# BarryFutureman/EvolutionaryDistributedTraining

Hardware: AMD Instinct MI355X
Metric: GB/s of param bytes reduced per outer step (device-resident), 1/2/4/8 GPUs (higher is better)
Workload: dtype f32; 1 GPU; DiLoCo outer step, gpt_1p3b P=1315723264 T=292, population 8 (8 f32 workers resident per GPU), f32 theta+momentum, lr 0.7 mu 0.9 nesterov True; params=1315723264, tensors=292, workers_per_gpu=8, population=8, worker_dtype=f32, theta_dtype=f32, parallelism=single GPU

## Files before the change

evolutionarydistributedtraining_amd/csrc/edt_common.h:

```cpp
#pragma once

#include <hip/hip_runtime.h>
#include <stdarg.h>
#include <stdint.h>
#include <stdio.h>
#include <string.h>

#include <type_traits>
#include <vector>

#include "edt_sync.h"

namespace edt {
extern thread_local char g_err[512];
}

namespace {
using edt::g_err;


#ifndef EDT_BLOCKS_PER_CU
#define EDT_BLOCKS_PER_CU 0
#endif
#ifndef EDT_NT_LOADS
#define EDT_NT_LOADS 1
#endif
#ifndef EDT_NT_RMW
#define EDT_NT_RMW 0
#endif
#ifndef EDT_NT_STORES
#define EDT_NT_STORES 0
#endif

#ifndef EDT_NT_LERP
#define EDT_NT_LERP 0
#endif
#ifndef EDT_NT_LERP_STORES
#define EDT_NT_LERP_STORES 1
#endif
#ifndef EDT_NT_SLERP_STORES
#define EDT_NT_SLERP_STORES 1
#endif
#ifndef EDT_NT_SLERP
#define EDT_NT_SLERP 1
#endif
#ifndef EDT_SLERP_STATS_TPW
#define EDT_SLERP_STATS_TPW 16
#endif
#ifndef EDT_GRAM_NT
#define EDT_GRAM_NT 1
#endif
#ifndef EDT_NEED_GROUP
#define EDT_NEED_GROUP 8
#endif
#ifndef EDT_NEED_MIN_WAVES
#define EDT_NEED_MIN_WAVES 1
#endif
#ifndef EDT_NEED_GLDS
#define EDT_NEED_GLDS 1
#endif
#ifndef EDT_SLERP_SPEC_WG_ROWS
#define EDT_SLERP_SPEC_WG_ROWS 1
#endif
#ifndef EDT_SLERP_COEF_BLOCK
#define EDT_SLERP_COEF_BLOCK 1
#endif
#ifndef EDT_SPLIT_HALVES
#define EDT_SPLIT_HALVES 2
#endif
#ifndef EDT_NT_F32
#define EDT_NT_F32 1
#endif
template <int WDT, int H2>
constexpr bool nt_worker_loads() {
    return EDT_NT_LOADS != 0 && (WDT == EDT_BF16 || (EDT_NT_F32 != 0 && H2 != 4));
}

template <int GDT, int WDT>
constexpr bool split_halves() {
    return EDT_SPLIT_HALVES == 1 || (EDT_SPLIT_HALVES == 2 && GDT == EDT_F32 && WDT == EDT_F32);
}
#ifndef EDT_MIN_WAVES
#define EDT_MIN_WAVES 1
#endif

constexpr int kBlock = 256;
constexpr int kVec = 8;
constexpr uint64_t kGridBlockCap = 0xffffffffull / kBlock;
constexpr uint64_t kMaxBlocks = EDT_BLOCKS_PER_CU > 0 ? 256ull * EDT_BLOCKS_PER_CU : kGridBlockCap;

#ifndef EDT_XCD_RUN
#define EDT_XCD_RUN 0
#endif
__device__ __forceinline__ uint64_t xcd_block(uint64_t b, uint64_t G) {
    if constexpr (EDT_XCD_RUN == 0) {
        return b;
    } else {
        const uint64_t M = EDT_XCD_RUN > 0 ? (uint64_t)EDT_XCD_RUN : G / 8;
        const uint64_t span = 8 * M;
        if (M == 0 || b >= G / span * span) return b;
        const uint64_t g = b / span, x = b % 8, j = (b / 8) % M;
        return g * span + x * M + j;
    }
}

#ifndef EDT_SLERP_SPEC_BPC
#define EDT_SLERP_SPEC_BPC 256
#endif
inline unsigned slerp_spec_grid(int64_t nchunks) {
    const uint64_t cap = 256ull * EDT_SLERP_SPEC_BPC;
    return (unsigned)((uint64_t)nchunks < cap ? (uint64_t)nchunks : cap);
}
typedef float f32x4 __attribute__((ext_vector_type(4)));
typedef float f32x2 __attribute__((ext_vector_type(2)));
typedef uint32_t u32x4 __attribute__((ext_vector_type(4)));
typedef uint32_t u32x2 __attribute__((ext_vector_type(2)));
typedef __bf16 bf16x2 __attribute__((ext_vector_type(2)));



inline int fail(int code, const char* fmt, ...) {
    va_list ap;
    va_start(ap, fmt);
    vsnprintf(g_err, sizeof(g_err), fmt, ap);
    va_end(ap);
    return code;
}

inline int check_launch(const char* what) {
    hipError_t e = hipGetLastError();
    if (e != hipSuccess) return fail(EDT_ERR_LAUNCH, "%s: launch failed: %s", what, hipGetErrorString(e));
    return EDT_OK;
}


__device__ __forceinline__ float bf_lo(uint32_t w) { return __uint_as_float(w << 16); }
__device__ __forceinline__ float bf_hi(uint32_t w) { return __uint_as_float(w & 0xffff0000u); }
__device__ __forceinline__ uint32_t pack_bf(float lo, float hi) {
    bf16x2 r = __builtin_convertvector((f32x2){lo, hi}, bf16x2);
    return __builtin_bit_cast(uint32_t, r);
}
__host__ __device__ inline float host_round_bf16(float x) {
    uint32_t u;
    memcpy(&u, &x, 4);
    if ((u & 0x7fffffffu) > 0x7f800000u) return x;
    u = (u + 0x7fffu + ((u >> 16) & 1u)) & 0xffff0000u;
    float r;
    memcpy(&r, &u, 4);
    return r;
}

template <int DT, int N>
__device__ __forceinline__ void rnd(float (&x)[N]) {
    if constexpr (DT == EDT_BF16) {
        if constexpr (N % 2 == 0) {
#pragma unroll
            for (int j = 0; j < N; j += 2) {
                uint32_t p = pack_bf(x[j], x[j + 1]);
                x[j] = bf_lo(p);
                x[j + 1] = bf_hi(p);
            }
        } else {
#pragma unroll
            for (int j = 0; j < N; ++j) x[j] = bf_lo(pack_bf(x[j], 0.f));
        }
    }
}

template <typename V, bool NT>
__device__ __forceinline__ V vload(const V* p) {
    if constexpr (NT) return __builtin_nontemporal_load(p);
    else return *p;
}
template <typename V, bool NT>
__device__ __forceinline__ void vstore(V* p, V v) {
    if constexpr (NT) __builtin_nontemporal_store(v, p);
    else *p = v;
}

template <int DT, int N, bool NT = false, int H2 = 4>
__device__ __forceinline__ void ld(const void* __restrict__ p, uint64_t i, float (&x)[N]) {
    if constexpr (DT == EDT_F32) {
        const float* q = static_cast<const float*>(p) + i;
        if constexpr (N == 8) {
            f32x4 a = vload<f32x4, NT>(reinterpret_cast<const f32x4*>(q));
            f32x4 b = vload<f32x4, NT>(reinterpret_cast<const f32x4*>(q + H2));
            x[0] = a.x; x[1] = a.y; x[2] = a.z; x[3] = a.w;
            x[4] = b.x; x[5] = b.y; x[6] = b.z; x[7] = b.w;
        } else {
#pragma unroll
            for (int j = 0; j < N; ++j) x[j] = q[j];
        }
    } else {
        const uint16_t* q = static_cast<const uint16_t*>(p) + i;
        if constexpr (N == 8 && H2 == 4) {
            u32x4 w = vload<u32x4, NT>(reinterpret_cast<const u32x4*>(q));
            x[0] = bf_lo(w.x); x[1] = bf_hi(w.x); x[2] = bf_lo(w.y); x[3] = bf_hi(w.y);
            x[4] = bf_lo(w.z); x[5] = bf_hi(w.z); x[6] = bf_lo(w.w); x[7] = bf_hi(w.w);
        } else if constexpr (N == 8) {
            u32x2 w0 = vload<u32x2, NT>(reinterpret_cast<const u32x2*>(q));
            u32x2 w1 = vload<u32x2, NT>(reinterpret_cast<const u32x2*>(q + H2));
            x[0] = bf_lo(w0.x); x[1] = bf_hi(w0.x); x[2] = bf_lo(w0.y); x[3] = bf_hi(w0.y);
            x[4] = bf_lo(w1.x); x[5] = bf_hi(w1.x); x[6] = bf_lo(w1.y); x[7] = bf_hi(w1.y);
        } else {
#pragma unroll
            for (int j = 0; j < N; ++j) x[j] = __uint_as_float(uint32_t(q[j]) << 16);
        }
    }
}

template <int DT, int N, bool NT = (EDT_NT_STORES != 0), int H2 = 4>
__device__ __forceinline__ void st(void* __restrict__ p, uint64_t i, const float (&x)[N]) {
    if constexpr (DT == EDT_F32) {
        float* q = static_cast<float*>(p) + i;
        if constexpr (N == 8) {
            vstore<f32x4, NT>(reinterpret_cast<f32x4*>(q), (f32x4){x[0], x[1], x[2], x[3]});
            vstore<f32x4, NT>(reinterpret_cast<f32x4*>(q + H2), (f32x4){x[4], x[5], x[6], x[7]});
        } else {
#pragma unroll
            for (int j = 0; j < N; ++j) q[j] = x[j];
        }
    } else {
        uint16_t* q = static_cast<uint16_t*>(p) + i;
        if constexpr (N == 8 && H2 == 4) {
            u32x4 w;
            w.x = pack_bf(x[0], x[1]); w.y = pack_bf(x[2], x[3]);
            w.z = pack_bf(x[4], x[5]); w.w = pack_bf(x[6], x[7]);
            vstore<u32x4, NT>(reinterpret_cast<u32x4*>(q), w);
        } else if constexpr (N == 8) {
            u32x2 w0, w1;
            w0.x = pack_bf(x[0], x[1]); w0.y = pack_bf(x[2], x[3]);
            w1.x = pack_bf(x[4], x[5]); w1.y = pack_bf(x[6], x[7]);
            vstore<u32x2, NT>(reinterpret_cast<u32x2*>(q), w0);
            vstore<u32x2, NT>(reinterpret_cast<u32x2*>(q + H2), w1);
        } else {
#pragma unroll
            for (int j = 0; j < N; ++j) q[j] = uint16_t(pack_bf(x[j], 0.f) & 0xffffu);
        }
    }
}


struct SgdScalars {
    float mul_mu;
    float alpha_mu;
    float alpha_nlr;
    int use_momentum;
    int has_buf;
    int nesterov;
    const uint8_t* tail;
};

inline SgdScalars make_sgd(int gdt, double lr, double mu, int has_buf, int nesterov) {
    SgdScalars s;
    s.mul_mu = (float)mu;
    s.alpha_mu = gdt == EDT_BF16 ? host_round_bf16((float)mu) : (float)mu;
    s.alpha_nlr = gdt == EDT_BF16 ? host_round_bf16((float)(-lr)) : (float)(-lr);
    s.use_momentum = mu != 0.0;
    s.has_buf = has_buf;
    s.nesterov = nesterov;
    s.tail = nullptr;
    return s;
}

template <int GDT, int N, int H2 = 4>
__device__ __forceinline__ void ld_momentum(const void* mom, uint64_t i, const SgdScalars& s, float (&b)[N]) {
    if (s.use_momentum && s.has_buf) ld<GDT, N, (EDT_NT_RMW != 0), H2>(mom, i, b);
}

__device__ __forceinline__ float tail_add(float x, float a, float y) {
    float p[1] = {a * y};
    rnd<EDT_BF16>(p);
    return x + p[0];
}

template <int GDT, int N, int H2 = 4>
__device__ __forceinline__ void sgd_update(float (&theta)[N], const float (&grad)[N], void* mom,
                                           uint64_t i, const SgdScalars& s, const float (&b_in)[N]) {
    uint32_t tb = 0;
    if constexpr (GDT == EDT_BF16 && H2 == 4 && (N == 8 || N == 1)) {
        if (s.tail) tb = N == 8 ? (uint32_t)s.tail[i >> 3] : ((uint32_t)s.tail[i >> 3] >> (i & 7)) & 1u;
    }
    float u[N];
    if (s.use_momentum) {
        float b[N];
        if (s.has_buf) {
#pragma unroll
            for (int j = 0; j < N; ++j) b[j] = b_in[j] * s.mul_mu;
            rnd<GDT>(b);
#pragma unroll
            for (int j = 0; j < N; ++j) b[j] = b[j] + grad[j];
            rnd<GDT>(b);
        } else {
#pragma unroll
            for (int j = 0; j < N; ++j) b[j] = grad[j];
        }
        st<GDT, N, (EDT_NT_STORES != 0), H2>(mom, i, b);
        if (s.nesterov) {
#pragma unroll
            for (int j = 0; j < N; ++j)
                u[j] = (tb >> j) & 1u ? tail_add(grad[j], s.alpha_mu, b[j]) : __builtin_fmaf(s.alpha_mu, b[j], grad[j]);
            rnd<GDT>(u);
        } else {
#pragma unroll
            for (int j = 0; j < N; ++j) u[j] = b[j];
        }
    } else {
#pragma unroll
        for (int j = 0; j < N; ++j) u[j] = grad[j];
    }
#pragma unroll
    for (int j = 0; j < N; ++j)
        theta[j] = (tb >> j) & 1u ? tail_add(theta[j], s.alpha_nlr, u[j]) : __builtin_fmaf(s.alpha_nlr, u[j], theta[j]);
    rnd<GDT>(theta);
}



template <int IDT, int ODT, int CDT, int N, bool NTL = false, bool NTS = (EDT_NT_STORES != 0)>
__device__ __forceinline__ void lerp_elems(const void* v0, const void* v1, void* out, uint64_t i,
                                           float c0, float c1) {
    float x[N], y[N];
    ld<IDT, N, NTL>(v0, i, x);
    ld<IDT, N, NTL>(v1, i, y);
#pragma unroll
    for (int j = 0; j < N; ++j) { x[j] = c0 * x[j]; y[j] = c1 * y[j]; }
    rnd<CDT>(x);
    rnd<CDT>(y);
#pragma unroll
    for (int j = 0; j < N; ++j) x[j] = x[j] + y[j];
    rnd<CDT>(x);
    st<ODT, N, NTS>(out, i, x);
}



inline bool aligned16(const void* p) { return (reinterpret_cast<uintptr_t>(p) & 15u) == 0; }

inline unsigned grid_for(uint64_t n, bool vec) {
    const uint64_t per = vec ? (uint64_t)kBlock * kVec : (uint64_t)kBlock;
    uint64_t g = (n + per - 1) / per;
    if (g < 1) g = 1;
    if (g > kMaxBlocks) g = kMaxBlocks;
    return (unsigned)g;
}

inline bool valid_pair(int gdt, int wdt) {
    return (gdt == EDT_F32 && (wdt == EDT_F32 || wdt == EDT_BF16)) || (gdt == EDT_BF16 && wdt == EDT_BF16);
}


inline bool is_pow2(int k) { return k > 0 && (k & (k - 1)) == 0; }

}
```

evolutionarydistributedtraining_amd/csrc/edt_outer.hip:

```cpp
#include "edt_common.h"

namespace {


struct Workers {
    const void* p[EDT_MAX_WORKERS];
};

struct OuterArgs {
    void* theta;
    void* mom;
    float* acc_out;
    uint64_t n;
    int K;
    float kdiv;
    float kinv;
    int div_exact;
    int accumulate;
    void* acc_ws;
    int acc_in;
    int acc_store;
    SgdScalars sgd;
    Workers w;
    Workers bc;
    int nbc;
    __device__ __forceinline__ const void* wp(int k) const { return w.p[k]; }
};

struct TensorArgs {
    void* theta;
    void* mom;
    float* acc_out;
    int K;
    float kdiv;
    float kinv;
    int accumulate;
    void* acc_ws;
    int acc_in;
    int acc_store;
    SgdScalars sgd;
    const void* const* w;
    uint64_t T;
    uint64_t t;
    __device__ __forceinline__ const void* wp(int k) const { return w[(uint64_t)k * T + t]; }
};

enum { MODE_FUSED = 0, MODE_PARTIAL = 1, MODE_CHAIN = 2 };

template <int GDT, int WDT, int KC, int DIV, int MODE, int N, class A, int H2 = 4, bool BC = false>
__device__ __forceinline__ void outer_elems(const A& a, uint64_t i) {
    float g[N], acc[N], b_in[N];
    ld<GDT, N, (EDT_NT_RMW != 0), H2>(a.theta, i, g);
    if constexpr (MODE != MODE_PARTIAL) ld_momentum<GDT, N, H2>(a.mom, i, a.sgd, b_in);
    if (MODE == MODE_PARTIAL && a.accumulate) {
        ld<EDT_F32, N, false, H2>(a.acc_out, i, acc);
    } else if (MODE == MODE_CHAIN && a.acc_in) {
        ld<GDT, N, false, H2>(a.acc_ws, i, acc);
    } else {
#pragma unroll
        for (int j = 0; j < N; ++j) acc[j] = 0.f;
    }
    const int K = KC > 0 ? KC : a.K;
    auto body = [&](int k) {
        float w[N];
        ld<WDT, N, nt_worker_loads<WDT, H2>(), H2>(a.wp(k), i, w);
#pragma unroll
        for (int j = 0; j < N; ++j) w[j] = w[j] - g[j];
        rnd<GDT>(w);
        if constexpr (DIV) {
#pragma unroll
            for (int j = 0; j < N; ++j) w[j] = w[j] / a.kdiv;
        } else {
#pragma unroll
            for (int j = 0; j < N; ++j) w[j] = w[j] * a.kinv;
        }
        rnd<GDT>(w);
#pragma unroll
        for (int j = 0; j < N; ++j) acc[j] = acc[j] + w[j];
        if constexpr (MODE != MODE_PARTIAL) rnd<GDT>(acc);
    };
    if constexpr (KC > 0) {
#pragma unroll
        for (int k = 0; k < KC; ++k) body(k);
    } else {
#pragma unroll 4
        for (int k = 0; k < K; ++k) body(k);
    }
    if constexpr (MODE == MODE_PARTIAL) {
        st<EDT_F32, N, (EDT_NT_STORES != 0), H2>(a.acc_out, i, acc);
    } else if (MODE == MODE_CHAIN && a.acc_store) {
        st<GDT, N, (EDT_NT_STORES != 0), H2>(a.acc_ws, i, acc);
    } else {
        float grad[N];
#pragma unroll
        for (int j = 0; j < N; ++j) grad[j] = -acc[j];
        sgd_update<GDT, N, H2>(g, grad, a.mom, i, a.sgd, b_in);
        st<GDT, N, (EDT_NT_STORES != 0), H2>(a.theta, i, g);
        if constexpr (BC) {
#pragma unroll 4
            for (int k = 0; k < a.nbc; ++k) st<WDT, N, (EDT_NT_STORES != 0), H2>(const_cast<void*>(a.bc.p[k]), i, g);
        }
    }
}

template <int GDT, int WDT, int KC, int DIV, int MODE, int N, bool BC = false>
__global__ __launch_bounds__(kBlock, EDT_MIN_WAVES) void outer_kernel(OuterArgs a) {
    const uint64_t stride = (uint64_t)gridDim.x * kBlock;
    const uint64_t tid = xcd_block(blockIdx.x, gridDim.x) * kBlock + threadIdx.x;
    if constexpr (N == kVec && split_halves<GDT, WDT>()) {
        constexpr int H2 = 4 * kBlock;
        const uint64_t nv = a.n / (kVec * kBlock) * kBlock;
        for (uint64_t v = tid; v < nv; v += stride)
            outer_elems<GDT, WDT, KC, DIV, MODE, kVec, OuterArgs, H2, BC>(a, v * kVec - 4 * threadIdx.x);
        for (uint64_t e = nv * kVec + tid; e < a.n; e += stride)
            outer_elems<GDT, WDT, KC, DIV, MODE, 1, OuterArgs, 4, BC>(a, e);
    } else if constexpr (N == kVec) {
        const uint64_t nv = a.n / kVec;
        for (uint64_t v = tid; v < nv; v += stride)
            outer_elems<GDT, WDT, KC, DIV, MODE, kVec, OuterArgs, 4, BC>(a, v * kVec);
        const uint64_t t = nv * kVec + tid;
        if (t < a.n) outer_elems<GDT, WDT, KC, DIV, MODE, 1, OuterArgs, 4, BC>(a, t);
    } else {
        for (uint64_t e = tid; e < a.n; e += stride) outer_elems<GDT, WDT, KC, DIV, MODE, 1, OuterArgs, 4, BC>(a, e);
    }
}

#ifndef EDT_LIST_ITERS
#define EDT_LIST_ITERS 2
#endif
constexpr uint64_t kListChunk = (uint64_t)kBlock * kVec * EDT_LIST_ITERS;
constexpr uint64_t kVecFlag = 1ull << 63;

struct ListArgs {
    const uint64_t* prefix;
    const uint64_t* numel;
    void* const* theta;
    void* const* mom;
    const void* const* w;
    uint64_t T;
    uint64_t chunks;
    int K;
    float kdiv;
    float kinv;
    SgdScalars sgd;
    const uint8_t* tail;
    const uint64_t* tail_off;
};

template <int GDT, int WDT, int KC, int DIV>
__device__ __forceinline__ void outer_list_chunk(const ListArgs& L, const uint64_t* prefix, uint64_t b) {
    uint64_t lo = 0, hi = L.T;
    while (hi - lo > 1) {
        const uint64_t mid = (lo + hi) >> 1;
        if (prefix[mid] <= b) lo = mid;
        else hi = mid;
    }
    const uint64_t t = lo;
    const uint64_t nf = L.numel[t];
    const uint64_t n = nf & ~kVecFlag;
    const uint64_t c0 = (b - prefix[t]) * kListChunk;
    const uint64_t c1 = c0 + kListChunk < n ? c0 + kListChunk : n;
    TensorArgs a;
    a.theta = L.theta[t];
    a.mom = L.sgd.use_momentum ? L.mom[t] : nullptr;
    a.acc_out = nullptr;
    a.K = L.K;
    a.kdiv = L.kdiv;
    a.kinv = L.kinv;
    a.accumulate = 0;
    a.acc_ws = nullptr;
    a.acc_in = 0;
    a.acc_store = 0;
    a.sgd = L.sgd;
    if (L.tail) a.sgd.tail = L.tail + L.tail_off[t];
    a.w = L.w;
    a.T = L.T;
    a.t = t;
    if ((nf & kVecFlag) && split_halves<GDT, WDT>()) {
        constexpr uint64_t tile = (uint64_t)kBlock * kVec;
        const uint64_t vend = c0 + (c1 - c0) / tile * tile;
        for (uint64_t i = c0 + 4ull * threadIdx.x; i < vend; i += tile)
            outer_elems<GDT, WDT, KC, DIV, MODE_FUSED, kVec, TensorArgs, 4 * kBlock>(a, i);
        for (uint64_t i = vend + threadIdx.x; i < c1; i += kBlock)
            outer_elems<GDT, WDT, KC, DIV, MODE_FUSED, 1>(a, i);
    } else if (nf & kVecFlag) {
        const uint64_t vend = c0 + (c1 - c0) / kVec * kVec;
        for (uint64_t i = c0 + (uint64_t)threadIdx.x * kVec; i < vend; i += (uint64_t)kBlock * kVec)
            outer_elems<GDT, WDT, KC, DIV, MODE_FUSED, kVec>(a, i);
        const uint64_t i = vend + threadIdx.x;
        if (i < c1) outer_elems<GDT, WDT, KC, DIV, MODE_FUSED, 1>(a, i);
    } else {
        for (uint64_t i = c0 + threadIdx.x; i < c1; i += kBlock)
            outer_elems<GDT, WDT, KC, DIV, MODE_FUSED, 1>(a, i);
    }
}

template <int GDT, int WDT, int KC, int DIV, bool LDS>
__global__ __launch_bounds__(kBlock, EDT_MIN_WAVES) void outer_list_kernel(ListArgs L) {
    extern __shared__ uint64_t s_prefix[];
    const uint64_t* prefix = L.prefix;
    if constexpr (LDS) {
        for (uint64_t i = threadIdx.x; i <= L.T; i += kBlock) s_prefix[i] = L.prefix[i];
        __syncthreads();
        prefix = s_prefix;
    }
    for (uint64_t b = blockIdx.x; b < L.chunks; b += gridDim.x) outer_list_chunk<GDT, WDT, KC, DIV>(L, prefix, b);
}

template <int GDT, int N>
__global__ __launch_bounds__(kBlock) void sgd_apply_kernel(void* theta, const float* acc, void* mom,
                                                           uint64_t n, SgdScalars s) {
    const uint64_t stride = (uint64_t)gridDim.x * kBlock;
    const uint64_t tid = (uint64_t)blockIdx.x * kBlock + threadIdx.x;
    auto elems = [&](auto tagN, uint64_t i) {
        constexpr int M = decltype(tagN)::value;
        float g[M], a[M], grad[M], b_in[M];
        ld<GDT, M>(theta, i, g);
        ld<EDT_F32, M>(acc, i, a);
        ld_momentum<GDT, M>(mom, i, s, b_in);
        rnd<GDT>(a);
#pragma unroll
        for (int j = 0; j < M; ++j) grad[j] = -a[j];
        sgd_update<GDT, M>(g, grad, mom, i, s, b_in);
        st<GDT, M>(theta, i, g);
    };
    using V8 = std::integral_constant<int, kVec>;
    using V1 = std::integral_constant<int, 1>;
    if constexpr (N == kVec) {
        const uint64_t nv = n / kVec;
        for (uint64_t v = tid; v < nv; v += stride) elems(V8{}, v * kVec);
        const uint64_t t = nv * kVec + tid;
        if (t < n) elems(V1{}, t);
    } else {
        for (uint64_t e = tid; e < n; e += stride) elems(V1{}, e);
    }
}


struct Partials {
    const float* p[EDT_MAX_WORKERS];
};

template <int GDT, int N>
__global__ __launch_bounds__(kBlock) void sgd_apply_sum_kernel(void* theta, Partials P, int np, void* mom,
                                                               uint64_t n, SgdScalars s) {
    const uint64_t stride = (uint64_t)gridDim.x * kBlock;
    const uint64_t tid = (uint64_t)blockIdx.x * kBlock + threadIdx.x;
    auto elems = [&](auto tagN, uint64_t i) {
        constexpr int M = decltype(tagN)::value;
        float g[M], a[M], grad[M], b_in[M];
        ld<GDT, M>(theta, i, g);
        ld_momentum<GDT, M>(mom, i, s, b_in);
        ld<EDT_F32, M>(P.p[0], i, a);
        for (int r = 1; r < np; ++r) {
            float x[M];
            ld<EDT_F32, M>(P.p[r], i, x);
#pragma unroll
            for (int j = 0; j < M; ++j) a[j] = a[j] + x[j];
        }
        rnd<GDT>(a);
#pragma unroll
        for (int j = 0; j < M; ++j) grad[j] = -a[j];
        sgd_update<GDT, M>(g, grad, mom, i, s, b_in);
        st<GDT, M>(theta, i, g);
    };
    using V8 = std::integral_constant<int, kVec>;
    using V1 = std::integral_constant<int, 1>;
    if constexpr (N == kVec) {
        const uint64_t nv = n / kVec;
        for (uint64_t v = tid; v < nv; v += stride) elems(V8{}, v * kVec);
        const uint64_t t = nv * kVec + tid;
        if (t < n) elems(V1{}, t);
    } else {
        for (uint64_t e = tid; e < n; e += stride) elems(V1{}, e);
    }
}



template <int GDT, int WDT, int KC, int N, int H2 = 4>
__device__ __forceinline__ void probe_elems(const OuterArgs& a, uint64_t i) {
    float g[N], b[N], acc[N];
    ld<GDT, N, false, H2>(a.theta, i, g);
    ld<GDT, N, false, H2>(a.mom, i, b);
#pragma unroll
    for (int j = 0; j < N; ++j) acc[j] = 0.f;
    const int K = KC > 0 ? KC : a.K;
#pragma unroll 8
    for (int k = 0; k < K; ++k) {
        float w[N];
        ld<WDT, N, nt_worker_loads<WDT, H2>(), H2>(a.wp(k), i, w);
#pragma unroll
        for (int j = 0; j < N; ++j) acc[j] += w[j];
    }
#pragma unroll
    for (int j = 0; j < N; ++j) { g[j] += acc[j] * 1e-30f; b[j] += acc[j] * 1e-30f; }
    st<GDT, N, (EDT_NT_STORES != 0), H2>(a.theta, i, g);
    st<GDT, N, (EDT_NT_STORES != 0), H2>(a.mom, i, b);
}

template <int GDT, int WDT, int KC>
__global__ __launch_bounds__(kBlock, EDT_MIN_WAVES) void probe_kernel(OuterArgs a) {
    const uint64_t stride = (uint64_t)gridDim.x * kBlock;
    const uint64_t tid = (uint64_t)blockIdx.x * kBlock + threadIdx.x;
    if constexpr (split_halves<GDT, WDT>()) {
        constexpr int H2 = 4 * kBlock;
        const uint64_t nv = a.n / (kVec * kBlock) * kBlock;
        for (uint64_t v = tid; v < nv; v += stride) probe_elems<GDT, WDT, KC, kVec, H2>(a, v * kVec - 4 * threadIdx.x);
        for (uint64_t e = nv * kVec + tid; e < a.n; e += stride) probe_elems<GDT, WDT, KC, 1>(a, e);
    } else {
        const uint64_t nv = a.n / kVec;
        for (uint64_t v = tid; v < nv; v += stride) probe_elems<GDT, WDT, KC, kVec>(a, v * kVec);
        const uint64_t t = nv * kVec + tid;
        if (t < a.n) probe_elems<GDT, WDT, KC, 1>(a, t);
    }
}



template <int GDT, int WDT, int MODE, bool BC = false>
int launch_outer_k(const OuterArgs& a, bool vec, hipStream_t s) {
    const unsigned g = grid_for(a.n, vec);
#define EDT_LAUNCH_K(KC, DIV)                                                                    \
    do {                                                                                         \
        if (vec) outer_kernel<GDT, WDT, KC, DIV, MODE, kVec, BC><<<g, kBlock, 0, s>>>(a);        \
        else outer_kernel<GDT, WDT, KC, DIV, MODE, 1, BC><<<g, kBlock, 0, s>>>(a);               \
    } while (0)
    if constexpr (MODE == MODE_CHAIN) {
        if (a.div_exact) EDT_LAUNCH_K(0, 1);
        else EDT_LAUNCH_K(0, 0);
        return check_launch("outer_kernel");
    }
    if (a.K == 1 && !a.div_exact) EDT_LAUNCH_K(1, 0);
    else if (a.K == 2 && !a.div_exact) EDT_LAUNCH_K(2, 0);
    else if (a.K == 3 && a.div_exact) EDT_LAUNCH_K(3, 1);
    else if (a.K == 4 && !a.div_exact) EDT_LAUNCH_K(4, 0);
    else if (a.K == 8 && !a.div_exact) EDT_LAUNCH_K(8, 0);
    else if (a.div_exact) EDT_LAUNCH_K(0, 1);
    else EDT_LAUNCH_K(0, 0);
#undef EDT_LAUNCH_K
    return check_launch("outer_kernel");
}

template <int MODE, bool BC = false>
int launch_outer(int gdt, int wdt, const OuterArgs& a, bool vec, hipStream_t s) {
    if (gdt == EDT_F32 && wdt == EDT_F32) return launch_outer_k<EDT_F32, EDT_F32, MODE, BC>(a, vec, s);
    if (gdt == EDT_F32 && wdt == EDT_BF16) return launch_outer_k<EDT_F32, EDT_BF16, MODE, BC>(a, vec, s);
    return launch_outer_k<EDT_BF16, EDT_BF16, MODE, BC>(a, vec, s);
}

constexpr uint64_t kListLdsMaxTensors = 8191;

template <int GDT, int WDT>
int launch_list_k(const ListArgs& L, int div_exact, unsigned grid, hipStream_t s) {
    const bool lds = L.T <= kListLdsMaxTensors;
    const size_t shm = lds ? (size_t)(L.T + 1) * sizeof(uint64_t) : 0;
#define EDT_LAUNCH_L(KC, DIV)                                                                    \
    do {                                                                                         \
        if (lds) outer_list_kernel<GDT, WDT, KC, DIV, true><<<grid, kBlock, shm, s>>>(L);        \
        else outer_list_kernel<GDT, WDT, KC, DIV, false><<<grid, kBlock, 0, s>>>(L);             \
    } while (0)
    if (L.K == 1 && !div_exact) EDT_LAUNCH_L(1, 0);
    else if (L.K == 2 && !div_exact) EDT_LAUNCH_L(2, 0);
    else if (L.K == 3 && div_exact) EDT_LAUNCH_L(3, 1);
    else if (L.K == 4 && !div_exact) EDT_LAUNCH_L(4, 0);
    else if (L.K == 8 && !div_exact) EDT_LAUNCH_L(8, 0);
    else if (div_exact) EDT_LAUNCH_L(0, 1);
    else EDT_LAUNCH_L(0, 0);
#undef EDT_LAUNCH_L
    return check_launch("outer_list_kernel");
}


int fill_outer(OuterArgs& a, const void* theta, const void* const* theta_k, int K, int K_total, uint64_t n) {
    memset(&a, 0, sizeof(a));
    if (!theta && n) return fail(EDT_ERR_ARG, "theta_g is null");
    if (K < 1 || K > EDT_MAX_WORKERS)
        return fail(EDT_ERR_ARG, "worker count %d out of range [1, %d]", K, EDT_MAX_WORKERS);
    if (K_total < 1) return fail(EDT_ERR_ARG, "total worker count %d < 1", K_total);
    if (!theta_k) return fail(EDT_ERR_ARG, "theta_k is null");
    for (int k = 0; k < K; ++k) {
        if (!theta_k[k] && n) return fail(EDT_ERR_ARG, "theta_k[%d] is null", k);
        a.w.p[k] = theta_k[k];
    }
    a.theta = const_cast<void*>(theta);
    a.n = n;
    a.K = K;
    a.kdiv = (float)K_total;
    a.kinv = 1.0f / (float)K_total;
    a.div_exact = is_pow2(K_total) ? 0 : 1;
    return EDT_OK;
}


}

extern "C" {

int edt_probe_stream(void* theta_g, int gdt, const void* const* theta_k, int wdt, int K, void* momentum,
                     uint64_t n, void* stream) {
    g_err[0] = 0;
    if (!valid_pair(gdt, wdt)) return fail(EDT_ERR_ARG, "unsupported dtype pair (gdt/wdt)");
    OuterArgs a;
    int rc = fill_outer(a, theta_g, theta_k, K, K, n);
    if (rc) return rc;
    if (!momentum) return fail(EDT_ERR_ARG, "momentum is null");
    a.mom = momentum;
    bool vec = aligned16(theta_g) && aligned16(momentum);
    for (int k = 0; k < K; ++k) vec = vec && aligned16(theta_k[k]);
    if (!vec) return fail(EDT_ERR_ARG, "the probe needs 16-byte aligned operands");
    if (n == 0) return EDT_OK;
    const unsigned g = grid_for(n, true);
    hipStream_t s = (hipStream_t)stream;
    if (gdt == EDT_F32 && wdt == EDT_BF16) {
        if (K == 8) probe_kernel<EDT_F32, EDT_BF16, 8><<<g, kBlock, 0, s>>>(a);
        else probe_kernel<EDT_F32, EDT_BF16, 0><<<g, kBlock, 0, s>>>(a);
    } else if (gdt == EDT_F32) {
        if (K == 8) probe_kernel<EDT_F32, EDT_F32, 8><<<g, kBlock, 0, s>>>(a);
        else probe_kernel<EDT_F32, EDT_F32, 0><<<g, kBlock, 0, s>>>(a);
    } else {
        if (K == 8) probe_kernel<EDT_BF16, EDT_BF16, 8><<<g, kBlock, 0, s>>>(a);
        else probe_kernel<EDT_BF16, EDT_BF16, 0><<<g, kBlock, 0, s>>>(a);
    }
    return check_launch("probe_kernel");
}

int edt_outer_step_bytes_per_elem(int gdt, int wdt, int K, int with_momentum) {
    const int bg = gdt == EDT_BF16 ? 2 : 4, bw = wdt == EDT_BF16 ? 2 : 4;
    return K * bw + 2 * bg + (with_momentum ? 2 * bg : 0);
}

int edt_outer_step(void* theta_g, int gdt, const void* const* theta_k, int wdt, int K,
                   void* momentum, int has_momentum, uint64_t n, double lr, double momentum_coef,
                   int nesterov, void* stream) {
    g_err[0] = 0;
    if (!valid_pair(gdt, wdt)) return fail(EDT_ERR_ARG, "unsupported dtype pair (gdt/wdt)");
    OuterArgs a;
    int rc = fill_outer(a, theta_g, theta_k, K, K, n);
    if (rc) return rc;
    a.sgd = make_sgd(gdt, lr, momentum_coef, has_momentum, nesterov);
    if (a.sgd.use_momentum && !momentum && n) return fail(EDT_ERR_ARG, "momentum buffer is null");
    a.mom = momentum;
    if (n == 0) return EDT_OK;
    bool vec = aligned16(theta_g) && (!a.sgd.use_momentum || aligned16(momentum));
    for (int k = 0; k < K; ++k) vec = vec && aligned16(theta_k[k]);
    return launch_outer<MODE_FUSED>(gdt, wdt, a, vec, (hipStream_t)stream);
}

int edt_outer_step_tail(void* theta_g, int gdt, const void* const* theta_k, int wdt, int K,
                        void* momentum, int has_momentum, uint64_t n, double lr, double momentum_coef,
                        int nesterov, const uint8_t* tail_bits, void* stream) {
    g_err[0] = 0;
    if (!valid_pair(gdt, wdt)) return fail(EDT_ERR_ARG, "unsupported dtype pair (gdt/wdt)");
    OuterArgs a;
    int rc = fill_outer(a, theta_g, theta_k, K, K, n);
    if (rc) return rc;
    a.sgd = make_sgd(gdt, lr, momentum_coef, has_momentum, nesterov);
    if (a.sgd.use_momentum && !momentum && n) return fail(EDT_ERR_ARG, "momentum buffer is null");
    a.mom = momentum;
    if (gdt == EDT_BF16) a.sgd.tail = tail_bits;
    if (n == 0) return EDT_OK;
    bool vec = aligned16(theta_g) && (!a.sgd.use_momentum || aligned16(momentum));
    for (int k = 0; k < K; ++k) vec = vec && aligned16(theta_k[k]);
    return launch_outer<MODE_FUSED>(gdt, wdt, a, vec, (hipStream_t)stream);
}

int edt_outer_step_bcast(void* theta_g, int gdt, const void* const* theta_k, int wdt, int K,
                         void* momentum, int has_momentum, uint64_t n, double lr, double momentum_coef,
                         int nesterov, void* const* bcast, int nbcast, void* stream) {
    g_err[0] = 0;
    if (!valid_pair(gdt, wdt)) return fail(EDT_ERR_ARG, "unsupported dtype pair (gdt/wdt)");
    if (nbcast < 0 || nbcast > EDT_MAX_WORKERS)
        return fail(EDT_ERR_ARG, "broadcast count %d out of range [0, %d]", nbcast, EDT_MAX_WORKERS);
    if (nbcast == 0)
        return edt_outer_step(theta_g, gdt, theta_k, wdt, K, momentum, has_momentum, n, lr, momentum_coef, nesterov,
                              stream);
    OuterArgs a;
    int rc = fill_outer(a, theta_g, theta_k, K, K, n);
    if (rc) return rc;
    a.sgd = make_sgd(gdt, lr, momentum_coef, has_momentum, nesterov);
    if (a.sgd.use_momentum && !momentum && n) return fail(EDT_ERR_ARG, "momentum buffer is null");
    a.mom = momentum;
    if (!bcast) return fail(EDT_ERR_ARG, "bcast is null");
    const uintptr_t t0 = reinterpret_cast<uintptr_t>(theta_g), t1 = t0 + n * (gdt == EDT_BF16 ? 2 : 4);
    for (int k = 0; k < nbcast; ++k) {
        if (!bcast[k] && n) return fail(EDT_ERR_ARG, "bcast[%d] is null", k);
        const uintptr_t b0 = reinterpret_cast<uintptr_t>(bcast[k]), b1 = b0 + n * (wdt == EDT_BF16 ? 2 : 4);
        if (n && b0 < t1 && t0 < b1) return fail(EDT_ERR_ARG, "bcast[%d] overlaps theta_g", k);
        a.bc.p[k] = bcast[k];
    }
    a.nbc = nbcast;
    if (n == 0) return EDT_OK;
    bool vec = aligned16(theta_g) && (!a.sgd.use_momentum || aligned16(momentum));
    for (int k = 0; k < K; ++k) vec = vec && aligned16(theta_k[k]);
    for (int k = 0; k < nbcast; ++k) vec = vec && aligned16(bcast[k]);
    return launch_outer<MODE_FUSED, true>(gdt, wdt, a, vec, (hipStream_t)stream);
}

int edt_outer_step_ws(void* theta_g, int gdt, const void* const* theta_k, int wdt, int K, void* momentum,
                      int has_momentum, uint64_t n, double lr, double momentum_coef, int nesterov, void* workspace,
                      void* stream) {
    if (K <= EDT_MAX_WORKERS)
        return edt_outer_step(theta_g, gdt, theta_k, wdt, K, momentum, has_momentum, n, lr, momentum_coef, nesterov,
                              stream);
    g_err[0] = 0;
    if (!valid_pair(gdt, wdt)) return fail(EDT_ERR_ARG, "unsupported dtype pair (gdt/wdt)");
    if (!workspace && n) return fail(EDT_ERR_ARG, "K = %d > %d needs a workspace of n elements of theta's dtype",
                                     K, EDT_MAX_WORKERS);
    if (!theta_k) return fail(EDT_ERR_ARG, "theta_k is null");
    const SgdScalars sg = make_sgd(gdt, lr, momentum_coef, has_momentum, nesterov);
    if (sg.use_momentum && !momentum && n) return fail(EDT_ERR_ARG, "momentum buffer is null");
    if (n == 0) return EDT_OK;
    bool vec = aligned16(theta_g) && aligned16(workspace) && (!sg.use_momentum || aligned16(momentum));
    for (int k = 0; k < K; ++k) vec = vec && theta_k[k] && aligned16(theta_k[k]);
    for (int k0 = 0; k0 < K; k0 += EDT_MAX_WORKERS) {
        const int kc = K - k0 < EDT_MAX_WORKERS ? K - k0 : EDT_MAX_WORKERS;
        OuterArgs a;
        int rc = fill_outer(a, theta_g, theta_k + k0, kc, K, n);
        if (rc) return rc;
        a.sgd = sg;
        a.mom = momentum;
        a.acc_ws = workspace;
        a.acc_in = k0 > 0;
        a.acc_store = k0 + kc < K;
        rc = launch_outer<MODE_CHAIN>(gdt, wdt, a, vec, (hipStream_t)stream);
        if (rc) return rc;
    }
    return EDT_OK;
}

uint64_t edt_outer_list_workspace_bytes(int T, int K) {
    if (T < 0 || K < 1) return 0;
    return (uint64_t)(5 * (uint64_t)T + 1 + (uint64_t)K * T) * sizeof(uint64_t);
}

}

static int outer_step_list_impl(void* const* theta_t, int gdt, const void* const* theta_k, int wdt, int K,
                                void* const* momentum_t, int has_momentum, const uint64_t* numel, int T,
                                double lr, double momentum_coef, int nesterov, const uint8_t* tail,
                                const uint64_t* tail_off, void* workspace, uint64_t workspace_bytes, void* stream) {
    g_err[0] = 0;
    if (!valid_pair(gdt, wdt)) return fail(EDT_ERR_ARG, "unsupported dtype pair (gdt/wdt)");
    if (K < 1 || K > EDT_MAX_WORKERS)
        return fail(EDT_ERR_ARG, "worker count %d out of range [1, %d]", K, EDT_MAX_WORKERS);
    if (T < 0) return fail(EDT_ERR_ARG, "tensor count %d < 0", T);
    if (T == 0) return EDT_OK;
    if (!theta_t || !theta_k || !numel) return fail(EDT_ERR_ARG, "null tensor table");
    const SgdScalars sg = make_sgd(gdt, lr, momentum_coef, has_momentum, nesterov);
    if (sg.use_momentum && !momentum_t) return fail(EDT_ERR_ARG, "momentum table is null");
    const uint64_t need = edt_outer_list_workspace_bytes(T, K);
    if (!workspace || workspace_bytes < need)
        return fail(EDT_ERR_ARG, "workspace of %llu bytes needed", (unsigned long long)need);
    if (reinterpret_cast<uintptr_t>(workspace) & 7u) return fail(EDT_ERR_ARG, "workspace must be 8-byte aligned");
    if (tail && (gdt != EDT_BF16 || !tail_off)) return fail(EDT_ERR_ARG, "tail bits need a bf16 master and byte offsets");
    thread_local std::vector<uint64_t> h;
    h.assign(need / sizeof(uint64_t), 0);
    uint64_t* prefix = h.data();
    uint64_t* nflag = prefix + T + 1;
    uint64_t* pth = nflag + T;
    uint64_t* pmo = pth + T;
    uint64_t* pw = pmo + T;
    uint64_t* ptail = pw + (uint64_t)K * T;
    if (tail)
        for (int t = 0; t < T; ++t) ptail[t] = tail_off[t];
    for (int t = 0; t < T; ++t) {
        const uint64_t n = numel[t];
        if (n >= kVecFlag) return fail(EDT_ERR_ARG, "tensor %d too large", t);
        bool vec = true;
        if (n) {
            if (!theta_t[t]) return fail(EDT_ERR_ARG, "theta_t[%d] is null", t);
            vec = aligned16(theta_t[t]);
            if (sg.use_momentum) {
                if (!momentum_t[t]) return fail(EDT_ERR_ARG, "momentum_t[%d] is null", t);
                vec = vec && aligned16(momentum_t[t]);
            }
            for (int k = 0; k < K; ++k) {
                const void* p = theta_k[(uint64_t)k * T + t];
                if (!p) return fail(EDT_ERR_ARG, "theta_k[%d][%d] is null", k, t);
                vec = vec && aligned16(p);
            }
        }
        prefix[t + 1] = prefix[t] + (n + kListChunk - 1) / kListChunk;
        nflag[t] = n | (vec ? kVecFlag : 0);
        pth[t] = reinterpret_cast<uintptr_t>(theta_t[t]);
        pmo[t] = sg.use_momentum ? reinterpret_cast<uintptr_t>(momentum_t[t]) : 0;
        for (int k = 0; k < K; ++k) pw[(uint64_t)k * T + t] = reinterpret_cast<uintptr_t>(theta_k[(uint64_t)k * T + t]);
    }
    const uint64_t chunks = prefix[T];
    if (chunks == 0) return EDT_OK;
    if (chunks > 0x7fffffffull) return fail(EDT_ERR_ARG, "too many elements for one launch");
    hipStream_t st = (hipStream_t)stream;
    hipError_t e = hipMemcpyAsync(workspace, h.data(), need, hipMemcpyHostToDevice, st);
    if (e != hipSuccess) return fail(EDT_ERR_LAUNCH, "tensor table upload failed: %s", hipGetErrorString(e));
    const uint64_t* d = static_cast<const uint64_t*>(workspace);
    ListArgs L;
    L.prefix = d;
    L.numel = d + T + 1;
    L.theta = reinterpret_cast<void* const*>(d + 2 * (uint64_t)T + 1);
    L.mom = reinterpret_cast<void* const*>(d + 3 * (uint64_t)T + 1);
    L.w = reinterpret_cast<const void* const*>(d + 4 * (uint64_t)T + 1);
    L.T = (uint64_t)T;
    L.chunks = chunks;
    L.K = K;
    L.kdiv = (float)K;
    L.kinv = 1.0f / (float)K;
    L.sgd = sg;
    L.tail = tail;
    L.tail_off = d + 4 * (uint64_t)T + 1 + (uint64_t)K * T;
    const int div_exact = is_pow2(K) ? 0 : 1;
    const unsigned grid = chunks > kMaxBlocks ? (unsigned)kMaxBlocks : (unsigned)chunks;
    if (gdt == EDT_F32 && wdt == EDT_F32) return launch_list_k<EDT_F32, EDT_F32>(L, div_exact, grid, st);
    if (gdt == EDT_F32) return launch_list_k<EDT_F32, EDT_BF16>(L, div_exact, grid, st);
    return launch_list_k<EDT_BF16, EDT_BF16>(L, div_exact, grid, st);
}

extern "C" {

int edt_outer_step_list(void* const* theta_t, int gdt, const void* const* theta_k, int wdt, int K,
                        void* const* momentum_t, int has_momentum, const uint64_t* numel, int T,
                        double lr, double momentum_coef, int nesterov, void* workspace,
                        uint64_t workspace_bytes, void* stream) {
    return outer_step_list_impl(theta_t, gdt, theta_k, wdt, K, momentum_t, has_momentum, numel, T, lr,
                                momentum_coef, nesterov, nullptr, nullptr, workspace, workspace_bytes, stream);
}

int edt_outer_step_list_tail(void* const* theta_t, int gdt, const void* const* theta_k, int wdt, int K,
                             void* const* momentum_t, int has_momentum, const uint64_t* numel, int T,
                             double lr, double momentum_coef, int nesterov, const uint8_t* tail_bits,
                             const uint64_t* tail_byte_offset, void* workspace, uint64_t workspace_bytes,
                             void* stream) {
    return outer_step_list_impl(theta_t, gdt, theta_k, wdt, K, momentum_t, has_momentum, numel, T, lr,
                                momentum_coef, nesterov, tail_bits, tail_byte_offset, workspace, workspace_bytes,
                                stream);
}

int edt_delta_partial(const void* theta_g, int gdt, const void* const* theta_k, int wdt, int K_local,
                      int K_total, uint64_t n, float* acc_f32, int accumulate, void* stream) {
    g_err[0] = 0;
    if (!valid_pair(gdt, wdt)) return fail(EDT_ERR_ARG, "unsupported dtype pair (gdt/wdt)");
    OuterArgs a;
    int rc = fill_outer(a, theta_g, theta_k, K_local, K_total, n);
    if (rc) return rc;
    if (!acc_f32 && n) return fail(EDT_ERR_ARG, "acc_f32 is null");
    a.acc_out = acc_f32;
    a.accumulate = accumulate;
    if (n == 0) return EDT_OK;
    bool vec = aligned16(theta_g) && aligned16(acc_f32);
    for (int k = 0; k < K_local; ++k) vec = vec && aligned16(theta_k[k]);
    return launch_outer<MODE_PARTIAL>(gdt, wdt, a, vec, (hipStream_t)stream);
}

int edt_sgd_apply_sum(void* theta_g, int gdt, const float* const* acc_f32, int nacc, void* momentum,
                      int has_momentum, uint64_t n, double lr, double momentum_coef, int nesterov, void* stream) {
    g_err[0] = 0;
    if (gdt != EDT_F32 && gdt != EDT_BF16) return fail(EDT_ERR_ARG, "unsupported dtype");
    if (nacc < 1 || nacc > EDT_MAX_WORKERS) return fail(EDT_ERR_ARG, "partial count %d out of range [1, %d]", nacc,
                                                         EDT_MAX_WORKERS);
    if (n == 0) return EDT_OK;
    if (!theta_g || !acc_f32) return fail(EDT_ERR_ARG, "null buffer");
    SgdScalars s = make_sgd(gdt, lr, momentum_coef, has_momentum, nesterov);
    if (s.use_momentum && !momentum) return fail(EDT_ERR_ARG, "momentum buffer is null");
    Partials P;
    memset(&P, 0, sizeof(P));
    bool vec = aligned16(theta_g) && (!s.use_momentum || aligned16(momentum));
    for (int r = 0; r < nacc; ++r) {
        if (!acc_f32[r]) return fail(EDT_ERR_ARG, "acc_f32[%d] is null", r);
        P.p[r] = acc_f32[r];
        vec = vec && aligned16(acc_f32[r]);
    }
    const unsigned g = grid_for(n, vec);
    hipStream_t st = (hipStream_t)stream;
    if (gdt == EDT_F32) {
        if (vec) sgd_apply_sum_kernel<EDT_F32, kVec><<<g, kBlock, 0, st>>>(theta_g, P, nacc, momentum, n, s);
        else sgd_apply_sum_kernel<EDT_F32, 1><<<g, kBlock, 0, st>>>(theta_g, P, nacc, momentum, n, s);
    } else {
        if (vec) sgd_apply_sum_kernel<EDT_BF16, kVec><<<g, kBlock, 0, st>>>(theta_g, P, nacc, momentum, n, s);
        else sgd_apply_sum_kernel<EDT_BF16, 1><<<g, kBlock, 0, st>>>(theta_g, P, nacc, momentum, n, s);
    }
    return check_launch("sgd_apply_sum_kernel");
}

int edt_sgd_apply(void* theta_g, int gdt, const float* acc_f32, void* momentum, int has_momentum,
                  uint64_t n, double lr, double momentum_coef, int nesterov, void* stream) {
    g_err[0] = 0;
    if (gdt != EDT_F32 && gdt != EDT_BF16) return fail(EDT_ERR_ARG, "unsupported dtype");
    if (n == 0) return EDT_OK;
    if (!theta_g || !acc_f32) return fail(EDT_ERR_ARG, "null buffer");
    SgdScalars s = make_sgd(gdt, lr, momentum_coef, has_momentum, nesterov);
    if (s.use_momentum && !momentum) return fail(EDT_ERR_ARG, "momentum buffer is null");
    const bool vec = aligned16(theta_g) && aligned16(acc_f32) && (!s.use_momentum || aligned16(momentum));
    const unsigned g = grid_for(n, vec);
    hipStream_t st = (hipStream_t)stream;
    if (gdt == EDT_F32) {
        if (vec) sgd_apply_kernel<EDT_F32, kVec><<<g, kBlock, 0, st>>>(theta_g, acc_f32, momentum, n, s);
        else sgd_apply_kernel<EDT_F32, 1><<<g, kBlock, 0, st>>>(theta_g, acc_f32, momentum, n, s);
    } else {
        if (vec) sgd_apply_kernel<EDT_BF16, kVec><<<g, kBlock, 0, st>>>(theta_g, acc_f32, momentum, n, s);
        else sgd_apply_kernel<EDT_BF16, 1><<<g, kBlock, 0, st>>>(theta_g, acc_f32, momentum, n, s);
    }
    return check_launch("sgd_apply_kernel");
}


}
```

Before: 4058 GB/s.

## Process two tiles per iteration with all loads issued before compute in f32 outer step

Adds a pipelined path for the f32/f32 fused outer kernel with a compile-time K: each block loads theta, momentum and all K worker vectors for two adjacent tiles, then uses a scheduling barrier before computing and storing both. The grid is halved to match. The aim is more memory requests in flight per thread, hiding latency in a bandwidth-bound reduction. It costs much higher register pressure (two tiles of K+2 vectors), which may reduce occupancy, and the probe kernel gets the same treatment.

```diff
diff --git a/evolutionarydistributedtraining_amd/csrc/edt_common.h b/evolutionarydistributedtraining_amd/csrc/edt_common.h
--- a/evolutionarydistributedtraining_amd/csrc/edt_common.h
+++ b/evolutionarydistributedtraining_amd/csrc/edt_common.h
@@ -80,6 +80,9 @@
 constexpr bool split_halves() {
     return EDT_SPLIT_HALVES == 1 || (EDT_SPLIT_HALVES == 2 && GDT == EDT_F32 && WDT == EDT_F32);
 }
+#ifndef EDT_OUTER_PIPE
+#define EDT_OUTER_PIPE 1
+#endif
 #ifndef EDT_MIN_WAVES
 #define EDT_MIN_WAVES 1
 #endif
diff --git a/evolutionarydistributedtraining_amd/csrc/edt_outer.hip b/evolutionarydistributedtraining_amd/csrc/edt_outer.hip
--- a/evolutionarydistributedtraining_amd/csrc/edt_outer.hip
+++ b/evolutionarydistributedtraining_amd/csrc/edt_outer.hip
@@ -103,11 +103,77 @@
     }
 }
 
+template <int KC>
+struct OuterTile {
+    float g[kVec], b_in[kVec], w[KC][kVec];
+};
+
+template <int GDT, int WDT, int KC, int H2>
+__device__ __forceinline__ void outer_load(const OuterArgs& a, uint64_t i, OuterTile<KC>& r) {
+    ld<GDT, kVec, (EDT_NT_RMW != 0), H2>(a.theta, i, r.g);
+    ld_momentum<GDT, kVec, H2>(a.mom, i, a.sgd, r.b_in);
+#pragma unroll
+    for (int k = 0; k < KC; ++k) ld<WDT, kVec, nt_worker_loads<WDT, H2>(), H2>(a.wp(k), i, r.w[k]);
+}
+
+template <int GDT, int KC, int DIV, int H2>
+__device__ __forceinline__ void outer_compute_store(const OuterArgs& a, uint64_t i, OuterTile<KC>& r) {
+    float acc[kVec], grad[kVec];
+#pragma unroll
+    for (int j = 0; j < kVec; ++j) acc[j] = 0.f;
+#pragma unroll
+    for (int k = 0; k < KC; ++k) {
+        float (&w)[kVec] = r.w[k];
+#pragma unroll
+        for (int j = 0; j < kVec; ++j) w[j] = w[j] - r.g[j];
+        rnd<GDT>(w);
+        if constexpr (DIV) {
+#pragma unroll
+            for (int j = 0; j < kVec; ++j) w[j] = w[j] / a.kdiv;
+        } else {
+#pragma unroll
+            for (int j = 0; j < kVec; ++j) w[j] = w[j] * a.kinv;
+        }
+        rnd<GDT>(w);
+#pragma unroll
+        for (int j = 0; j < kVec; ++j) acc[j] = acc[j] + w[j];
+        rnd<GDT>(acc);
+    }
+#pragma unroll
+    for (int j = 0; j < kVec; ++j) grad[j] = -acc[j];
+    sgd_update<GDT, kVec, H2>(r.g, grad, a.mom, i, a.sgd, r.b_in);
+    st<GDT, kVec, (EDT_NT_STORES != 0), H2>(a.theta, i, r.g);
+}
+
+template <int GDT, int WDT, int KC, int MODE, int N, bool BC>
+constexpr bool outer_pipe() {
+    return EDT_OUTER_PIPE != 0 && N == kVec && GDT == EDT_F32 && WDT == EDT_F32 && split_halves<GDT, WDT>() &&
+           MODE == MODE_FUSED && !BC && KC > 0;
+}
+
 template <int GDT, int WDT, int KC, int DIV, int MODE, int N, bool BC = false>
 __global__ __launch_bounds__(kBlock, EDT_MIN_WAVES) void outer_kernel(OuterArgs a) {
     const uint64_t stride = (uint64_t)gridDim.x * kBlock;
     const uint64_t tid = xcd_block(blockIdx.x, gridDim.x) * kBlock + threadIdx.x;
-    if constexpr (N == kVec && split_halves<GDT, WDT>()) {
+    if constexpr (outer_pipe<GDT, WDT, KC, MODE, N, BC>()) {
+        constexpr int H2 = 4 * kBlock;
+        constexpr uint64_t tile = (uint64_t)kVec * kBlock;
+        const uint64_t tiles = a.n / tile, pairs = tiles / 2;
+        const uint64_t blk = xcd_block(blockIdx.x, gridDim.x);
+        for (uint64_t p = blk; p < pairs; p += gridDim.x) {
+            const uint64_t i = 2 * p * tile + 4 * threadIdx.x;
+            OuterTile<KC> ra, rb;
+            outer_load<GDT, WDT, KC, H2>(a, i, ra);
+            outer_load<GDT, WDT, KC, H2>(a, i + tile, rb);
+            __builtin_amdgcn_sched_barrier(0);
+            outer_compute_store<GDT, KC, DIV, H2>(a, i, ra);
+            outer_compute_store<GDT, KC, DIV, H2>(a, i + tile, rb);
+        }
+        if ((tiles & 1) && blk == pairs % gridDim.x)
+            outer_elems<GDT, WDT, KC, DIV, MODE, kVec, OuterArgs, H2, BC>(a, 2 * pairs * tile + 4 * threadIdx.x);
+        for (uint64_t e = tiles * tile + tid; e < a.n; e += stride)
+            outer_elems<GDT, WDT, KC, DIV, MODE, 1, OuterArgs, 4, BC>(a, e);
+    } else if constexpr (N == kVec && split_halves<GDT, WDT>()) {
         constexpr int H2 = 4 * kBlock;
         const uint64_t nv = a.n / (kVec * kBlock) * kBlock;
         for (uint64_t v = tid; v < nv; v += stride)
@@ -299,11 +365,51 @@
     st<GDT, N, (EDT_NT_STORES != 0), H2>(a.mom, i, b);
 }
 
+template <int GDT, int WDT, int KC, int H2>
+__device__ __forceinline__ void probe_load(const OuterArgs& a, uint64_t i, OuterTile<KC>& r) {
+    ld<GDT, kVec, false, H2>(a.theta, i, r.g);
+    ld<GDT, kVec, false, H2>(a.mom, i, r.b_in);
+#pragma unroll
+    for (int k = 0; k < KC; ++k) ld<WDT, kVec, nt_worker_loads<WDT, H2>(), H2>(a.wp(k), i, r.w[k]);
+}
+
+template <int GDT, int WDT, int KC, int H2>
+__device__ __forceinline__ void probe_store(const OuterArgs& a, uint64_t i, OuterTile<KC>& r) {
+    float acc[kVec];
+#pragma unroll
+    for (int j = 0; j < kVec; ++j) acc[j] = 0.f;
+#pragma unroll
+    for (int k = 0; k < KC; ++k) {
+#pragma unroll
+        for (int j = 0; j < kVec; ++j) acc[j] += r.w[k][j];
+    }
+#pragma unroll
+    for (int j = 0; j < kVec; ++j) { r.g[j] += acc[j] * 1e-30f; r.b_in[j] += acc[j] * 1e-30f; }
+    st<GDT, kVec, (EDT_NT_STORES != 0), H2>(a.theta, i, r.g);
+    st<GDT, kVec, (EDT_NT_STORES != 0), H2>(a.mom, i, r.b_in);
+}
+
 template <int GDT, int WDT, int KC>
 __global__ __launch_bounds__(kBlock, EDT_MIN_WAVES) void probe_kernel(OuterArgs a) {
     const uint64_t stride = (uint64_t)gridDim.x * kBlock;
     const uint64_t tid = (uint64_t)blockIdx.x * kBlock + threadIdx.x;
-    if constexpr (split_halves<GDT, WDT>()) {
+    if constexpr (outer_pipe<GDT, WDT, KC, MODE_FUSED, kVec, false>()) {
+        constexpr int H2 = 4 * kBlock;
+        constexpr uint64_t tile = (uint64_t)kVec * kBlock;
+        const uint64_t tiles = a.n / tile, pairs = tiles / 2;
+        for (uint64_t p = blockIdx.x; p < pairs; p += gridDim.x) {
+            const uint64_t i = 2 * p * tile + 4 * threadIdx.x;
+            OuterTile<KC> ra, rb;
+            probe_load<GDT, WDT, KC, H2>(a, i, ra);
+            probe_load<GDT, WDT, KC, H2>(a, i + tile, rb);
+            __builtin_amdgcn_sched_barrier(0);
+            probe_store<GDT, WDT, KC, H2>(a, i, ra);
+            probe_store<GDT, WDT, KC, H2>(a, i + tile, rb);
+        }
+        if ((tiles & 1) && blockIdx.x == pairs % gridDim.x)
+            probe_elems<GDT, WDT, KC, kVec, H2>(a, 2 * pairs * tile + 4 * threadIdx.x);
+        for (uint64_t e = tiles * tile + tid; e < a.n; e += stride) probe_elems<GDT, WDT, KC, 1>(a, e);
+    } else if constexpr (split_halves<GDT, WDT>()) {
         constexpr int H2 = 4 * kBlock;
         const uint64_t nv = a.n / (kVec * kBlock) * kBlock;
         for (uint64_t v = tid; v < nv; v += stride) probe_elems<GDT, WDT, KC, kVec, H2>(a, v * kVec - 4 * threadIdx.x);
@@ -323,7 +429,9 @@
     const unsigned g = grid_for(a.n, vec);
 #define EDT_LAUNCH_K(KC, DIV)                                                                    \
     do {                                                                                         \
-        if (vec) outer_kernel<GDT, WDT, KC, DIV, MODE, kVec, BC><<<g, kBlock, 0, s>>>(a);        \
+        if (vec)                                                                                 \
+            outer_kernel<GDT, WDT, KC, DIV, MODE, kVec, BC>                                      \
+                <<<outer_pipe<GDT, WDT, KC, MODE, kVec, BC>() ? (g + 1) / 2 : g, kBlock, 0, s>>>(a); \
         else outer_kernel<GDT, WDT, KC, DIV, MODE, 1, BC><<<g, kBlock, 0, s>>>(a);               \
     } while (0)
     if constexpr (MODE == MODE_CHAIN) {
@@ -416,7 +524,8 @@
         if (K == 8) probe_kernel<EDT_F32, EDT_BF16, 8><<<g, kBlock, 0, s>>>(a);
         else probe_kernel<EDT_F32, EDT_BF16, 0><<<g, kBlock, 0, s>>>(a);
     } else if (gdt == EDT_F32) {
-        if (K == 8) probe_kernel<EDT_F32, EDT_F32, 8><<<g, kBlock, 0, s>>>(a);
+        constexpr bool pipe = outer_pipe<EDT_F32, EDT_F32, 8, MODE_FUSED, kVec, false>();
+        if (K == 8) probe_kernel<EDT_F32, EDT_F32, 8><<<pipe ? (g + 1) / 2 : g, kBlock, 0, s>>>(a);
         else probe_kernel<EDT_F32, EDT_F32, 0><<<g, kBlock, 0, s>>>(a);
     } else {
         if (K == 8) probe_kernel<EDT_BF16, EDT_BF16, 8><<<g, kBlock, 0, s>>>(a);
```

Result: no change. 4075 GB/s (median of 4 runs) (+0.4%).
